# mmurooka/SMPLpp

Hardware: AMD Instinct MI355X
Metric: SMPL FK evals/s + IK iters/s, batch 1024 frames, 1/2/4/8 MI355X (higher is better)
Workload: dtype f32 (exact operands: every fp32 value as three bf16 pieces = fp32's 24 bits on the bf16 matrix pipe, fp32 accumulate; fp32 VALU skinning)

## Files before the change

### smplpp_amd/csrc/skin_h.hip

```cpp
#include "common.h"
#include "fk_launch.h"
#include "slot_pipe.h"

namespace smplpp_hip
{
typedef float f32x16 __attribute__((ext_vector_type(16)));
typedef float v3f __attribute__((ext_vector_type(3), aligned(4)));
typedef float v4f __attribute__((ext_vector_type(4)));
typedef unsigned v3u __attribute__((ext_vector_type(3)));
typedef _Float16 f16x8 __attribute__((ext_vector_type(8)));

constexpr int H_R = 7;
constexpr int H_LDS_RING = HB_G_BYTES;
constexpr int H_LDS_TR = H_LDS_RING + H_R * HB_IMG;
constexpr int H_LDS_TOTAL = H_LDS_TR + 64 * 16;

constexpr int wrap15(int u)
{
  return u < 0 ? u + HB_SLOTS : u;
}
constexpr int h_tail_slot(int k)
{
  return k <= 4 ? k : (k == 5 ? 4 : (k <= 10 ? k - 1 : (k == 11 ? 9 : k - 2)));
}
constexpr int h_tail_m(int k)
{
  return (k == 5 || k == 11) ? 8 : 5;
}
constexpr int h_tail_rows_in(int u)
{
  int c = 0;
  for(int k = 0; k < 16; k++) c += h_tail_slot(k) == u;
  return c;
}
constexpr int h_after_dma(int u, bool ht, bool rest)
{
  return u < 14 ? (ht ? h_tail_rows_in(u) : (u < 9 ? 2 : 0)) : ((u == 14 && rest) ? 16 : 0);
}
constexpr int h_slot_ops(int u, bool ht, bool rest)
{
  return 3 + h_after_dma(u, ht, rest);
}
constexpr int h_barrier_vmcnt(int s, bool ht, bool rest)
{
  if(!ht && s == 13) return 12;
  int c = s - 6 < 0 ? ((wrap15(s - 6) == 14 && rest && ht) ? 16 : 0) : h_after_dma(s - 6, ht, rest);
  for(int u = s - 5; u < s; u++) c += u < 0 ? 3 + ((wrap15(u) == 14 && rest && ht) ? 16 : 0) : h_slot_ops(u, ht, rest);
  return c < 63 ? c : 63;
}
static_assert(h_tail_rows_in(4) == 2 && h_tail_rows_in(9) == 2 && h_tail_rows_in(13) == 1 && h_tail_rows_in(14) == 0, "tail placement");
static_assert(h_barrier_vmcnt(0, false, true) == 15 && h_barrier_vmcnt(1, false, false) == 12 + 5 && h_barrier_vmcnt(0, true, true) == 31 &&
                  h_barrier_vmcnt(1, true, false) == 5 * 3 + 1 && h_barrier_vmcnt(8, true, false) == 15 + 7 && h_barrier_vmcnt(14, false, false) == 2 + 15,
              "window bookkeeping");

#ifndef SKINH_STORE_AUX
#define SKINH_STORE_AUX 0
#endif
#ifndef SKINH_DMA_IMM
#define SKINH_DMA_IMM 1
#endif
#ifndef SKINH_ABL
#define SKINH_ABL 0
#endif
#if SKINH_ABL & (256 | 512)
__device__ unsigned long long g_hslot_times[8 * 256];
__device__ unsigned long long g_hwg_times[256 * 4];
#endif

template<bool WANT_REST>
__global__ __launch_bounds__(256, 1) void skin_kernel_h(const uint8_t * __restrict__ A2h, const uint8_t * __restrict__ B2h,
                                                        const uint8_t * __restrict__ G2h, const float * __restrict__ theta,
                                                        float * __restrict__ verts, float * __restrict__ rest, int64_t n,
                                                        int64_t V, int nvg, int nft, float cAB)
{
  extern __shared__ __attribute__((aligned(16))) unsigned char lds[];
  typedef __attribute__((address_space(3))) void * lds_ptr_t;
  const int tid = threadIdx.x, lane = tid & 63, half = lane >> 5, l31 = lane & 31;
  const int wave = __builtin_amdgcn_readfirstlane(tid >> 6), wf = wave & 1, wv = wave >> 1;
  const XcdRun run = xcd_run(gridDim.x, blockIdx.x, nvg, nft);
  const int vg0 = run.vg0, vg1 = run.vg1, nvx = run.nvx, i0 = run.i0, i1 = run.i1;
  if(i0 >= i1) return;

#if SKINH_ABL & 512
  const unsigned long long t_start = __builtin_amdgcn_s_memtime(), r_start = __builtin_amdgcn_s_memrealtime();
#endif
  const int frameB = (int)(V * 12);
  const __amdgpu_buffer_rsrc_t rsB =
      __builtin_amdgcn_make_buffer_rsrc(const_cast<uint8_t *>(B2h), 0, (int)(nvg * HB_SLOTS * HB_IMG), 0x00020000);
  const __amdgpu_buffer_rsrc_t rsG =
      __builtin_amdgcn_make_buffer_rsrc(const_cast<uint8_t *>(G2h), 0, (int)(nft * HB_G_BYTES), 0x00020000);
  const __amdgpu_buffer_rsrc_t rsV = __builtin_amdgcn_make_buffer_rsrc(verts, 0, (int)(verts ? n * V * 12 : 0), 0x00020000);
  const __amdgpu_buffer_rsrc_t rsR = __builtin_amdgcn_make_buffer_rsrc(rest, 0, (int)(rest ? n * V * 12 : 0), 0x00020000);
  const int voffDma = wave * 3072 + lane * 16;

  const unsigned char * imgV[H_R];
  int imgS[H_R];
#pragma unroll
  for(int k = 0; k < H_R; k++)
  {
    imgS[k] = H_LDS_RING + k * HB_IMG;
    imgV[k] = lds + imgS[k] + wv * 6144 + lane * 16;
  }
  const unsigned char * const gLane0 = lds + wf * (12 * 3072) + lane * 16;
  const unsigned char * const gLane1 = lds + wf * (12 * 3072) + 2048 + l31 * 16;
  const unsigned char * const trLane = lds + H_LDS_TR + (wf * 32 + 4 * half) * 16;

#if SKINH_ABL & (256 | 512)
  int dbg_item = 0;
#endif
  f32x16 acc[3], macc[3];
  float tt[3][16];
  v4f areg[HB_KS][2];
  v4f bfr[2][3][2];
  v4f gfr[2][4];
  v4f wfr[4];
  v4f trb[2];
  const f32x16 zero16 = {0.f, 0.f, 0.f, 0.f, 0.f, 0.f, 0.f, 0.f, 0.f, 0.f, 0.f, 0.f, 0.f, 0.f, 0.f, 0.f};

  struct Item
  {
    int voff;
    int sb;
    float cw;
  } cur = {0x7fffff00, 0, 0.f}, prev = {0x7fffff00, 0, 0.f};

  auto mfma = [](const v4f & a, const v4f & b, const f32x16 & c) {
    return __builtin_amdgcn_mfma_f32_32x32x16_f16(__builtin_bit_cast(f16x8, a), __builtin_bit_cast(f16x8, b), c, 0, 0, 0);
  };
  auto dma = [&](auto itag, int vgBase, int slot, int dst) {
    constexpr int I = decltype(itag)::value;
    if constexpr(SKINH_ABL & 2) return;
#if SKINH_DMA_IMM
    __builtin_amdgcn_raw_ptr_buffer_load_lds(rsB, (lds_ptr_t)(lds + dst + wave * 3072), 16, voffDma, vgBase + slot * HB_IMG, I * 1024, 0);
#else
    __builtin_amdgcn_raw_ptr_buffer_load_lds(rsB, (lds_ptr_t)(lds + dst + wave * 3072 + I * 1024), 16, voffDma,
                                             vgBase + slot * HB_IMG + I * 1024, 0, 0);
#endif
  };

  v3f ovh;
  auto tail_prep = [&](auto rtag) {
    constexpr int R = decltype(rtag)::value;
    const v4f tr = trb[R & 1];
    if constexpr(R + 1 < 16) trb[(R + 1) & 1] = *reinterpret_cast<const v4f *>(trLane + ((((R + 1) & 3) + 8 * ((R + 1) >> 2)) * 16));
    const float u = __builtin_fmaf(tt[2][R], cAB, macc[2][R]);
    ovh = v3f{__builtin_fmaf(tt[0][R], prev.cw, tr.x), __builtin_fmaf(tt[1][R], prev.cw, tr.y), __builtin_fmaf(u, prev.cw, tr.z)};
  };
  auto tail_store = [&](auto rtag) {
    constexpr int R = decltype(rtag)::value;
    constexpr int ROWC = (R & 3) + 8 * (R >> 2);
    if constexpr(SKINH_ABL & 32)
    {
      const float o0 = ovh.x, o1 = ovh.y, o2 = ovh.z;
      asm volatile("" ::"v"(o0), "v"(o1), "v"(o2));
    }
    else
      __builtin_amdgcn_raw_buffer_store_b96(__builtin_bit_cast(v3u, ovh), rsV, prev.voff, prev.sb + ROWC * frameB, SKINH_STORE_AUX);
    asm volatile("s_nop 1");
  };
  auto tail_row = [&](auto rtag) {
    tail_prep(rtag);
    tail_store(rtag);
  };
  auto standalone_tail = [&]() {
    static_for<16>([&](auto rr) {
      tail_row(rr);
      SCHED_BARRIER();
    });
  };

  auto load_frame_tile = [&](int ft, auto first_tag) {
    constexpr bool FIRST = decltype(first_tag)::value;
    full_barrier();
#if SKINH_ABL & 512
    if(FIRST && blockIdx.x == 8 && tid == 0) g_hslot_times[70] = __builtin_amdgcn_s_memtime();
#endif
    float tval = 0.0f;
    if(tid < 192)
    {
      const int64_t f = (int64_t)ft * 64 + tid / 3;
      if(f < n) tval = theta[f * ((NJ + 1) * 3) + tid % 3];
    }
    const int vgF = vg0 + i0 % nvx;
    if constexpr(FIRST)
    {
      dma(std::integral_constant<int, 0>{}, vgF * (HB_SLOTS * HB_IMG), 0, imgS[0]);
      dma(std::integral_constant<int, 1>{}, vgF * (HB_SLOTS * HB_IMG), 0, imgS[0]);
      dma(std::integral_constant<int, 2>{}, vgF * (HB_SLOTS * HB_IMG), 0, imgS[0]);
    }
    const uint8_t * ap = A2h + ((int64_t)ft * HB_KS * 2 + wf) * 2048 + lane * 16;
#pragma unroll
    for(int ks = 0; ks < HB_KS; ks++)
#pragma unroll
      for(int p = 0; p < 2; p++) areg[ks][p] = *reinterpret_cast<const v4f *>(ap + ks * HB_A_BYTES + p * 1024);
    if constexpr(FIRST)
      static_for<H_R - 1>([&](auto dd) {
        constexpr int D = decltype(dd)::value + 1;
        dma(std::integral_constant<int, 0>{}, vgF * (HB_SLOTS * HB_IMG), D, imgS[D]);
        dma(std::integral_constant<int, 1>{}, vgF * (HB_SLOTS * HB_IMG), D, imgS[D]);
        dma(std::integral_constant<int, 2>{}, vgF * (HB_SLOTS * HB_IMG), D, imgS[D]);
      });
    if constexpr(FIRST)
    {
      waitcnt_barrier<28 + 18, 0, !(SKINH_ABL & 1)>();
#pragma unroll
      for(int q = 0; q < 6; q++) bfr[0][q / 2][q % 2] = *reinterpret_cast<const v4f *>(imgV[0] + q * 1024);
    }
    if(tid < 192) *reinterpret_cast<float *>(lds + H_LDS_TR + (tid / 3) * 16 + (tid % 3) * 4) = tval;
#if SKINH_ABL & 512
    if(FIRST && blockIdx.x == 8 && tid == 0) g_hslot_times[72] = __builtin_amdgcn_s_memtime();
#endif
  };

  auto do_item = [&](int ft_in, int vg_in, int vgn_in, auto ht_tag) {
    constexpr bool HT = decltype(ht_tag)::value;
    const int ft = __builtin_amdgcn_readfirstlane(ft_in), vg = __builtin_amdgcn_readfirstlane(vg_in), vgn = __builtin_amdgcn_readfirstlane(vgn_in);
    const int Bcur = vg * (HB_SLOTS * HB_IMG), Bnext = vgn * (HB_SLOTS * HB_IMG);
    cur.sb = __builtin_amdgcn_readfirstlane((ft * 64 + wf * 32) * frameB);
    int gcls = 3;

#if SKINH_ABL & 512
    if(blockIdx.x == 8 && tid == 0 && dbg_item < 8)
    {
      g_hslot_times[dbg_item * 8 + 0] = __builtin_amdgcn_s_memtime();
      g_hslot_times[dbg_item * 8 + 1] = __builtin_amdgcn_s_memrealtime();
    }
#endif
    static_for<HB_KS>([&](auto ss) {
      constexpr int S = decltype(ss)::value;
      static_for<9>([&](auto mm) {
        constexpr int M = decltype(mm)::value, X = M / 3, Q = M % 3;
        const v4f & a = areg[S][Q == 2 ? 1 : 0];
        const v4f & b = bfr[S & 1][X][Q == 1 ? 1 : 0];
#if SKINH_ABL & 256
        if(blockIdx.x == 0 && tid == 0 && dbg_item < 8) g_hslot_times[dbg_item * 256 + S * 9 + M] = __builtin_readcyclecounter();
#endif
#if SKINH_ABL & 512
        if(M == 0 && S < 8 && blockIdx.x == 8 && tid == 0 && dbg_item == 0) g_hslot_times[80 + S] = __builtin_amdgcn_s_memtime();
#endif
        if constexpr(SKINH_ABL & 4)
        {
          if constexpr(S == 0 && Q == 0) acc[X] = zero16;
          asm volatile("" ::"v"(a), "v"(b));
        }
        else if constexpr(S == 0 && Q == 0)
          acc[X] = mfma(a, b, zero16);
        else
          acc[X] = mfma(a, b, acc[X]);
        SCHED_BARRIER();
        if constexpr(M == 1) waitcnt_barrier<h_barrier_vmcnt(S, HT, WANT_REST), 0, !(SKINH_ABL & 1)>();
        if constexpr(M >= 2 && M <= 4)
          dma(std::integral_constant<int, M - 2>{}, S + 7 < HB_SLOTS ? Bcur : Bnext, S + 7 < HB_SLOTS ? S + 7 : S + 7 - HB_SLOTS,
              imgS[S % H_R]);
        if constexpr(!HT && S < 9 && (M == 5 || M == 6))
        {
          constexpr int PC = (2 * S + (M - 5)) * 4;
          __builtin_amdgcn_raw_ptr_buffer_load_lds(rsG, (lds_ptr_t)(lds + (PC + wave) * 1024), 16, lane * 16,
                                                   ft * HB_G_BYTES + (PC + wave) * 1024, 0, 0);
        }
        if constexpr(HT && (M == 5 || M == 7))
          static_for<16>([&](auto kk) {
            constexpr int K = decltype(kk)::value;
            if constexpr(h_tail_slot(K) == S && h_tail_m(K) == (M == 5 ? 5 : 8)) tail_prep(kk);
          });
        if constexpr(HT && (M == 6 || M == 8))
          static_for<16>([&](auto kk) {
            constexpr int K = decltype(kk)::value;
            if constexpr(h_tail_slot(K) == S && h_tail_m(K) == (M == 6 ? 5 : 8)) tail_store(kk);
          });
        if constexpr(S < HB_KS - 1 && M >= 2 && M <= 4 && !(SKINH_ABL & 16))
        {
          bfr[(S + 1) & 1][M - 2][0] = *reinterpret_cast<const v4f *>(imgV[(S + 1) % H_R] + (2 * (M - 2)) * 1024);
          bfr[(S + 1) & 1][M - 2][1] = *reinterpret_cast<const v4f *>(imgV[(S + 1) % H_R] + (2 * (M - 2) + 1) * 1024);
        }
        if constexpr(S == HB_KS - 1)
        {
          const unsigned char * wimg = imgV[HB_KS % H_R] - wv * 4096;
          if constexpr(M >= 2 && M <= 5) wfr[M - 2] = *reinterpret_cast<const v4f *>(wimg + ((M - 2) / 2) * 4096 + ((M - 2) % 2) * 1024);
          if constexpr(M == 6)
          {
            cur.cw = *reinterpret_cast<const float *>(lds + imgS[HB_KS % H_R] + HB_CW_OFF + (wv * 32 + l31) * 4);
            const int pv = *reinterpret_cast<const int *>(lds + imgS[HB_KS % H_R] + HB_PERM_OFF + (wv * 32 + l31) * 4);
            cur.voff = pv >= 0 ? pv * 12 + (4 * half) * frameB : 0x7fffff00;
            gcls = __builtin_amdgcn_readfirstlane(*reinterpret_cast<const int *>(lds + imgS[HB_KS % H_R] + HB_FLAGS_OFF));
          }
          if constexpr(M == 7)
          {
            gfr[0][0] = *reinterpret_cast<const v4f *>(gLane0);
            gfr[0][1] = *reinterpret_cast<const v4f *>(gLane0 + 1024);
          }
          if constexpr(M == 8)
          {
            gfr[0][2] = *reinterpret_cast<const v4f *>(gLane1);
            gfr[0][3] = *reinterpret_cast<const v4f *>(gLane1 + 512);
          }
        }
        SCHED_BARRIER();
      });
    });

#if SKINH_ABL & 512
    if(blockIdx.x == 8 && tid == 0 && dbg_item < 8)
    {
      g_hslot_times[dbg_item * 8 + 2] = __builtin_amdgcn_s_memtime();
      g_hslot_times[dbg_item * 8 + 3] = __builtin_amdgcn_s_memrealtime();
    }
#endif
    auto skin_phase = [&](auto ctag) {
    constexpr int CLS = decltype(ctag)::value;
    constexpr bool K0 = (CLS & 1) != 0, K1 = (CLS & 2) != 0;
    static_for<12>([&](auto ee) {
      constexpr int E = decltype(ee)::value, MPE = E & 1, ME = E % 3;
      static_for<5>([&](auto bb) {
        constexpr int B = decltype(bb)::value;
        constexpr bool LIVE = (B == 0 || B == 1 || B == 3) ? K0 : K1;
        constexpr int FIRST = K0 ? 0 : 2;
        constexpr int GI = B < 2 ? 0 : (B == 2 ? 2 : (B == 3 ? 1 : 3));
        constexpr int WI = B == 0 ? 0 : (B == 1 ? 1 : (B == 2 ? 3 : (B == 3 ? 0 : 2)));
#if SKINH_ABL & 256
        if(blockIdx.x == 0 && tid == 0 && dbg_item < 8) g_hslot_times[dbg_item * 256 + 126 + E * 5 + B] = __builtin_readcyclecounter();
#endif
        if constexpr(SKINH_ABL & 8)
        {
          if constexpr(B == 0) macc[ME] = zero16;
        }
        else if constexpr(!LIVE)
          ;
        else if constexpr(B == FIRST)
          macc[ME] = mfma(gfr[MPE][GI], wfr[WI], zero16);
        else
          macc[ME] = mfma(gfr[MPE][GI], wfr[WI], macc[ME]);
        SCHED_BARRIER();
        if constexpr(E == 0 && B == 0) waitcnt_barrier<h_barrier_vmcnt(HB_KS, HT, WANT_REST), 0, !(SKINH_ABL & 1)>();
        if constexpr(E == 0 && B >= 1 && B <= 3) dma(std::integral_constant<int, B - 1>{}, Bnext, HB_KS + 7 - HB_SLOTS, imgS[HB_KS % H_R]);
        if constexpr(E == 1)
        {
          bfr[0][B / 2][B % 2] = *reinterpret_cast<const v4f *>(imgV[(HB_KS + 1) % H_R] + B * 1024);
          if constexpr(B == 4) bfr[0][2][1] = *reinterpret_cast<const v4f *>(imgV[(HB_KS + 1) % H_R] + 5 * 1024);
        }
        if constexpr(E < 11 && B <= 3 && !(SKINH_ABL & (8 | 16)))
        {
          constexpr int I = B == 0 ? 0 : (B == 1 ? 2 : (B == 2 ? 1 : 3));
          if constexpr(I < 2 ? K0 : K1)
            gfr[MPE ^ 1][I] = *reinterpret_cast<const v4f *>((I < 2 ? gLane0 + I * 1024 : gLane1 + (I - 2) * 512) + (E + 1) * 3072);
        }
        if constexpr(E == 11 && B == 4)
          trb[0] = *reinterpret_cast<const v4f *>(trLane);
        auto blend_rows = [&](auto ftag, auto r0tag, auto r1tag) {
          constexpr int F = decltype(ftag)::value, XF = F / 4, CF = F % 4, MF = F % 3, R0 = decltype(r0tag)::value, R1 = decltype(r1tag)::value;
#pragma unroll
          for(int r = R0; r < R1; r++)
          {
            if constexpr(CF == 0) tt[XF][r] = macc[MF][r] * acc[0][r];
            if constexpr(CF == 1) tt[XF][r] = __builtin_fmaf(macc[MF][r], acc[1][r], tt[XF][r]);
            if constexpr(CF == 2) tt[XF][r] = __builtin_fmaf(macc[MF][r], acc[2][r], tt[XF][r]);
            if constexpr(CF == 3) tt[XF][r] = __builtin_fmaf(tt[XF][r], cAB, macc[MF][r]);
          }
        };
        if constexpr(!(SKINH_ABL & 8))
        {
          if constexpr(E >= 1 && B >= 1)
            blend_rows(std::integral_constant<int, E - 1>{}, std::integral_constant<int, 3 * (B - 1)>{}, std::integral_constant<int, 3 * B>{});
          if constexpr(E >= 2 && B == 0)
            blend_rows(std::integral_constant<int, E - 2>{}, std::integral_constant<int, 12>{}, std::integral_constant<int, 16>{});
          if constexpr(E == 11 && B == 4)
            blend_rows(std::integral_constant<int, 10>{}, std::integral_constant<int, 12>{}, std::integral_constant<int, 16>{});
        }
        if constexpr(WANT_REST && E >= 2 && E <= 9 && B < 2)
        {
          constexpr int R = 2 * (E - 2) + B, ROWC = (R & 3) + 8 * (R >> 2);
          v3f ov = {acc[0][R] * cAB, acc[1][R] * cAB, acc[2][R] * cAB};
          __builtin_amdgcn_raw_buffer_store_b96(__builtin_bit_cast(v3u, ov), rsR, cur.voff, cur.sb + ROWC * frameB, SKINH_STORE_AUX);
          asm volatile("s_nop 1");
        }
        SCHED_BARRIER();
      });
    });
    };
    if(gcls == 1)
      skin_phase(std::integral_constant<int, 1>{});
    else if(gcls == 2)
      skin_phase(std::integral_constant<int, 2>{});
    else
      skin_phase(std::integral_constant<int, 3>{});

    prev = cur;
#if SKINH_ABL & (256 | 512)
    dbg_item++;
#endif
    {
      const unsigned char * v0 = imgV[0];
      const int s0 = imgS[0];
#pragma unroll
      for(int k = 0; k < H_R - 1; k++)
      {
        imgV[k] = imgV[k + 1];
        imgS[k] = imgS[k + 1];
      }
      imgV[H_R - 1] = v0;
      imgS[H_R - 1] = s0;
    }
  };

  for(int i = i0; i < i1;)
  {
    const int ft = i / nvx;
    const int iend = (ft + 1) * nvx < i1 ? (ft + 1) * nvx : i1;
    if(i != i0)
    {
      standalone_tail();
      load_frame_tile(ft, std::false_type{});
    }
    else
      load_frame_tile(ft, std::true_type{});
    int vgk = vg0 + (i - ft * nvx);
    auto next_vg = [&](int k, int vgc) { return k + 1 < i1 ? (vgc + 1 < vg1 ? vgc + 1 : vg0) : vgc; };
    do_item(ft, vgk, next_vg(i, vgk), std::false_type{});
    for(int k = i + 1; k < iend; k++)
    {
      vgk++;
      do_item(ft, vgk, next_vg(k, vgk), std::true_type{});
    }
    i = iend;
  }
  standalone_tail();
#if SKINH_ABL & 512
  if(blockIdx.x == 8 && tid == 0)
  {
    g_hslot_times[64] = __builtin_amdgcn_s_memtime();
    g_hslot_times[65] = __builtin_amdgcn_s_memrealtime();
    g_hslot_times[66] = t_start;
    g_hslot_times[67] = r_start;
    g_hslot_times[68] = i1 - i0;
  }
  if(tid == 0 && blockIdx.x < 256)
  {
    g_hwg_times[blockIdx.x * 4 + 0] = r_start;
    g_hwg_times[blockIdx.x * 4 + 1] = __builtin_amdgcn_s_memrealtime();
    g_hwg_times[blockIdx.x * 4 + 2] = __builtin_amdgcn_s_memtime() - t_start;
    g_hwg_times[blockIdx.x * 4 + 3] = (unsigned long long)(i1 - i0) | ((unsigned long long)__builtin_amdgcn_s_getreg((6 << 11) | 20) << 32);
  }
#endif
  asm volatile("s_waitcnt vmcnt(0)" ::: "memory");
}

static hipError_t launch_h(const smplpp_model * m, const SkinBatch & b, hipStream_t st)
{
  const int nft = (int)((b.n + 63) / 64);
  const int nvg = (int)m->VGPn;
  const int nbx = skin_grid(device_cus(m->device), nvg, nft, true);
  const bool wr = b.rest != nullptr;
  static PerDeviceOnce once[2];
  {
    hipError_t e = lds_opt_in(once[wr], m->device, wr ? reinterpret_cast<const void *>(&skin_kernel_h<true>) : reinterpret_cast<const void *>(&skin_kernel_h<false>), H_LDS_TOTAL);
    if(e != hipSuccess) return e;
  }
  const float cAB = 1.0f / (HB_SA * m->sB);
  const uint8_t * A2 = b.tiles<uint8_t>(m->ws.A2h, HB_KS * HB_A_BYTES), * G2 = b.tiles<uint8_t>(m->ws.G2h, HB_G_BYTES);
  if(wr)
    skin_kernel_h<true><<<dim3(nbx * 8), dim3(256), H_LDS_TOTAL, st>>>(A2, m->B2h.get(), G2, b.theta, b.verts, b.rest, b.n, m->V, nvg, nft, cAB);
  else
    skin_kernel_h<false><<<dim3(nbx * 8), dim3(256), H_LDS_TOTAL, st>>>(A2, m->B2h.get(), G2, b.theta, b.verts, b.rest, b.n, m->V, nvg, nft, cAB);
  return hipGetLastError();
}

#if SKINH_ABL & (256 | 512)
extern "C" int smplpp_debug_hwg_times(unsigned long long * out)
{
  return (int)hipMemcpyFromSymbol(out, HIP_SYMBOL(smplpp_hip::g_hwg_times), sizeof(unsigned long long) * 256 * 4);
}
extern "C" int smplpp_debug_hslot_times(unsigned long long * out)
{
  return (int)hipMemcpyFromSymbol(out, HIP_SYMBOL(smplpp_hip::g_hslot_times), sizeof(unsigned long long) * 8 * 256);
}
#endif
hipError_t launch_skin_f16x2(const smplpp_model * m, int64_t n, const float * theta, float * verts, float * rest, hipStream_t st)
{
  return for_each_skin_batch(m->V, n, HB_G_BYTES, theta, verts, rest, [&](const SkinBatch & b) { return launch_h(m, b, st); });
}
}
```

Measured before the change: 15.38 million.

## Keep trailing G fragments register-resident across items instead of reloading from LDS

Adds a register array holding the later G-matrix fragment entries for the skinning MFMAs. With the default resident sizes, the last 10 (or 7 with rest output) entries are loaded from LDS only once, in the head-tile path, and then reused across items. Only the leading entries keep streaming through the double-buffered fragments. This cuts per-item LDS reads in the blend phase but raises VGPR pressure considerably (up to 48 v4f), which risks spills at launch bounds of 256 with one block.

```diff
diff --git a/smplpp_amd/csrc/skin_h.hip b/smplpp_amd/csrc/skin_h.hip
--- a/smplpp_amd/csrc/skin_h.hip
+++ b/smplpp_amd/csrc/skin_h.hip
@@ -62,6 +62,20 @@
 #ifndef SKINH_ABL
 #define SKINH_ABL 0
 #endif
+#ifndef SKINH_G_RESIDENT
+#define SKINH_G_RESIDENT 40
+#endif
+#ifndef SKINH_G_RESIDENT_REST
+#define SKINH_G_RESIDENT_REST 28
+#endif
+constexpr int h_g_lds_entries(bool rest)
+{
+  return (48 - (rest ? SKINH_G_RESIDENT_REST : SKINH_G_RESIDENT)) / 4;
+}
+static_assert(SKINH_G_RESIDENT % 4 == 0 && SKINH_G_RESIDENT >= 0 && SKINH_G_RESIDENT <= 48 && SKINH_G_RESIDENT_REST % 4 == 0 &&
+                  SKINH_G_RESIDENT_REST >= 0 && SKINH_G_RESIDENT_REST <= 48,
+              "the resident set is whole entries (4 fragments each) of the 12");
+
 #if SKINH_ABL & (256 | 512)
 __device__ unsigned long long g_hslot_times[8 * 256];
 __device__ unsigned long long g_hwg_times[256 * 4];
@@ -113,6 +127,8 @@
   v4f areg[HB_KS][2];
   v4f bfr[2][3][2];
   v4f gfr[2][4];
+  constexpr int NLE = h_g_lds_entries(WANT_REST);
+  v4f gres[12][4];
   v4f wfr[4];
   v4f trb[2];
   const f32x16 zero16 = {0.f, 0.f, 0.f, 0.f, 0.f, 0.f, 0.f, 0.f, 0.f, 0.f, 0.f, 0.f, 0.f, 0.f, 0.f, 0.f};
@@ -284,15 +300,15 @@
             cur.voff = pv >= 0 ? pv * 12 + (4 * half) * frameB : 0x7fffff00;
             gcls = __builtin_amdgcn_readfirstlane(*reinterpret_cast<const int *>(lds + imgS[HB_KS % H_R] + HB_FLAGS_OFF));
           }
-          if constexpr(M == 7)
+          if constexpr(M == 7 && (NLE > 0 || !HT))
           {
-            gfr[0][0] = *reinterpret_cast<const v4f *>(gLane0);
-            gfr[0][1] = *reinterpret_cast<const v4f *>(gLane0 + 1024);
+            (NLE > 0 ? gfr[0][0] : gres[0][0]) = *reinterpret_cast<const v4f *>(gLane0);
+            (NLE > 0 ? gfr[0][1] : gres[0][1]) = *reinterpret_cast<const v4f *>(gLane0 + 1024);
           }
-          if constexpr(M == 8)
+          if constexpr(M == 8 && (NLE > 0 || !HT))
           {
-            gfr[0][2] = *reinterpret_cast<const v4f *>(gLane1);
-            gfr[0][3] = *reinterpret_cast<const v4f *>(gLane1 + 512);
+            (NLE > 0 ? gfr[0][2] : gres[0][2]) = *reinterpret_cast<const v4f *>(gLane1);
+            (NLE > 0 ? gfr[0][3] : gres[0][3]) = *reinterpret_cast<const v4f *>(gLane1 + 512);
           }
         }
         SCHED_BARRIER();
@@ -327,9 +343,9 @@
         else if constexpr(!LIVE)
           ;
         else if constexpr(B == FIRST)
-          macc[ME] = mfma(gfr[MPE][GI], wfr[WI], zero16);
+          macc[ME] = mfma(E < NLE ? gfr[MPE][GI] : gres[E][GI], wfr[WI], zero16);
         else
-          macc[ME] = mfma(gfr[MPE][GI], wfr[WI], macc[ME]);
+          macc[ME] = mfma(E < NLE ? gfr[MPE][GI] : gres[E][GI], wfr[WI], macc[ME]);
         SCHED_BARRIER();
         if constexpr(E == 0 && B == 0) waitcnt_barrier<h_barrier_vmcnt(HB_KS, HT, WANT_REST), 0, !(SKINH_ABL & 1)>();
         if constexpr(E == 0 && B >= 1 && B <= 3) dma(std::integral_constant<int, B - 1>{}, Bnext, HB_KS + 7 - HB_SLOTS, imgS[HB_KS % H_R]);
@@ -341,8 +357,13 @@
         if constexpr(E < 11 && B <= 3 && !(SKINH_ABL & (8 | 16)))
         {
           constexpr int I = B == 0 ? 0 : (B == 1 ? 2 : (B == 2 ? 1 : 3));
-          if constexpr(I < 2 ? K0 : K1)
-            gfr[MPE ^ 1][I] = *reinterpret_cast<const v4f *>((I < 2 ? gLane0 + I * 1024 : gLane1 + (I - 2) * 512) + (E + 1) * 3072);
+          const unsigned char * const gsrc = (I < 2 ? gLane0 + I * 1024 : gLane1 + (I - 2) * 512) + (E + 1) * 3072;
+          if constexpr(E + 1 < NLE)
+          {
+            if constexpr(I < 2 ? K0 : K1) gfr[MPE ^ 1][I] = *reinterpret_cast<const v4f *>(gsrc);
+          }
+          else if constexpr(!HT)
+            gres[E + 1][I] = *reinterpret_cast<const v4f *>(gsrc);
         }
         if constexpr(E == 11 && B == 4)
           trb[0] = *reinterpret_cast<const v4f *>(trLane);
```

New measurement: 15.41 million (median of 3 runs). No clear change (+0.2%).
